# aymenboudhina/Multimodal_VQVAE_compression_audio_tactile

Measured on AMD Instinct MI355X. Metric: encode+VQ+decode token-frames/sec (1 frame = 13.33 ms of paired 24 kHz audio+tactile), higher is better.
Workload: dtype f32

## Files before the change

### multimodal_vqvae_compression_audio_tactile_amd/csrc/conv1d_mfma.hpp

```cpp
#pragma once
#include <hip/hip_runtime.h>
#include <stdio.h>
#include <stdlib.h>
#include <type_traits>
#include "det_math.hpp"
#include "kernels_small.hpp"

namespace mvq {

struct ConvArgs;
inline bool conv_dma_rows_ok(const ConvArgs& a);

__device__ __attribute__((aligned(16))) static const float g_zero16[4] = {0.0f, 0.0f, 0.0f, 0.0f};

int prof_begin(const char* kernel_name, double flops, hipStream_t s);
void prof_end(int idx, hipStream_t s);
bool prof_enabled();

typedef float f32x16 __attribute__((ext_vector_type(16)));
typedef float f32x4 __attribute__((ext_vector_type(4)));

struct ConvArgs {
    const float* x;
    const float* wp;
// ... 215 lines not shown
    static_assert(WAVES_M * WAVES_N == 4 || WAVES_M * WAVES_N == 8, "block is 4 or 8 waves");
    static_assert(KC % 2 == 0, "chunk K must be even (32x32x2 MFMA)");
    static_assert(BM % 4 == 0, "float4 weight staging");
};

template <int KS, int STRIDE, int DIL, int CK, int MT, int NT, int WAVES_M, int WAVES_N, int UPS, bool VEC>
struct ConvTile {
    using C = ConvCfg<KS, STRIDE, DIL, CK, MT, NT, WAVES_M, WAVES_N, UPS>;
    const float* wp; const float* xb; const float* Al;
    float* Ws; float* Xs;
    int tid, Tin, Cin, Mpad, m0, t_in0, g_al;
    bool snake_in;

    __device__ __forceinline__ void load_chunk(int chunk, f32x4 (&wreg)[C::W_PER_THREAD], f32x4 (&xv)[C::XV_PER_THREAD], float (&xs)[C::XS_PER_THREAD]) const
    {
        const int ci0 = chunk * CK;
        const float* wsrc = wp + (size_t)ci0 * KS * Mpad + m0;
#pragma unroll
        for (int u = 0; u < C::W_PER_THREAD; ++u) {
            int v = tid + u * C::NTHR;
            if (C::W_VEC % C::NTHR != 0) v = v < C::W_VEC ? v : C::W_VEC - 1;
            const int row = v / (C::BM / 4);
            const int c4 = v - row * (C::BM / 4);
            wreg[u] = *reinterpret_cast<const f32x4*>(wsrc + (size_t)row * Mpad + c4 * 4);
        }
        if (VEC) {
#pragma unroll
            for (int u = 0; u < C::XV_PER_THREAD; ++u) {
                int e = tid + u * C::NTHR;
                if (C::XV_TOTAL % C::NTHR != 0) e = e < C::XV_TOTAL ? e : C::XV_TOTAL - 1;
                const int cl = e / C::XV;
                const int v = e - cl * C::XV;
                const int g = g_al + 4 * v;
                const bool ok = g >= 0 && g < Tin;
                const int gc = ok ? g : 0;
                xv[u] = *reinterpret_cast<const f32x4*>(xb + (size_t)(ci0 + cl) * Tin + gc);
            }
        } else {
#pragma unroll
            for (int u = 0; u < C::XS_PER_THREAD; ++u) {
                int e = tid + u * C::NTHR;
                if (C::XS_TOTAL % C::NTHR != 0) e = e < C::XS_TOTAL ? e : C::XS_TOTAL - 1;
                const int cl = e / C::XT;
                const int xi = e - cl * C::XT;
                const int g = t_in0 + xi;
                const bool ok = g >= 0 && g < Tin;
                const int gc = ok ? g : 0;
                xs[u] = xb[(size_t)(ci0 + cl) * Tin + gc];
            }
        }
    }

    __device__ __forceinline__ void store_chunk(int chunk, int buf, const f32x4 (&wreg)[C::W_PER_THREAD],
                                                const f32x4 (&xv)[C::XV_PER_THREAD],
                                                const float (&xs)[C::XS_PER_THREAD]) const
    {
        const int ci0 = chunk * CK;
        float* wdst = Ws + buf * C::W_FLOATS;
        float* xdst = Xs + buf * C::X_FLOATS;
#pragma unroll
        for (int u = 0; u < C::W_PER_THREAD; ++u) {
            const int v = tid + u * C::NTHR;
            if (C::W_VEC % C::NTHR == 0 || v < C::W_VEC) *reinterpret_cast<f32x4*>(wdst + v * 4) = wreg[u];
        }
        if (VEC) {
#pragma unroll
            for (int u = 0; u < C::XV_PER_THREAD; ++u) {
                const int e = tid + u * C::NTHR;
                const int ec = (C::XV_TOTAL % C::NTHR != 0 && e >= C::XV_TOTAL) ? C::XV_TOTAL - 1 : e;
                const int cl = ec / C::XV;
                const int v = ec - cl * C::XV;
                const int g = g_al + 4 * v;
                const bool ok = g >= 0 && g < Tin;
                f32x4 q = xv[u];
                if (!ok) q = f32x4{0.0f, 0.0f, 0.0f, 0.0f};
                if (snake_in) {
                    const float al = Al[ci0 + cl], inv = Al[Cin + ci0 + cl];
                    q.x = det_snake(q.x, al, inv); q.y = det_snake(q.y, al, inv);
                    q.z = det_snake(q.z, al, inv); q.w = det_snake(q.w, al, inv);
                }
                if (C::XV_TOTAL % C::NTHR == 0 || e < C::XV_TOTAL)
                    *reinterpret_cast<f32x4*>(xdst + cl * C::XTP + 4 * v) = q;
            }
        } else {
#pragma unroll
            for (int u = 0; u < C::XS_PER_THREAD; ++u) {
                const int e = tid + u * C::NTHR;
                const int ec = (C::XS_TOTAL % C::NTHR != 0 && e >= C::XS_TOTAL) ? C::XS_TOTAL - 1 : e;
                const int cl = ec / C::XT;
                const int xi = ec - cl * C::XT;
                const int g = t_in0 + xi;
                float q = (g >= 0 && g < Tin) ? xs[u] : 0.0f;
                if (snake_in) q = det_snake(q, Al[ci0 + cl], Al[Cin + ci0 + cl]);
                if (C::XS_TOTAL % C::NTHR == 0 || e < C::XS_TOTAL) xdst[cl * C::XTP + xi] = q;
            }
        }
    }
};

template <int KS, int STRIDE, int DIL, int CK, int MT, int NT, int WAVES_M, int WAVES_N, int UPS, bool VEC, bool FUSE>
__device__ __forceinline__ void conv1d_mfma_body(const ConvArgs& a)
{
    using C = ConvCfg<KS, STRIDE, DIL, CK, MT, NT, WAVES_M, WAVES_N, UPS>;
    extern __shared__ __attribute__((aligned(16))) float smem[];
    float* const Ws = smem;
    float* const Xs = smem + 2 * C::W_FLOATS;
    float* const Ep = smem + (FUSE ? (a.dma ? C::LDS_FLOATS_FUSE_DMA : C::LDS_FLOATS_FUSE) : (a.dma ? C::LDS_FLOATS_DMA : C::LDS_FLOATS));
    constexpr int EP_MID = 2;
    float* const Al = Ep + 3 * C::BM;

    const int tid = threadIdx.x;
    const int lane = tid & 63;
    const int wave = tid >> 6;
    const int wm = wave / WAVES_N;
    const int wn = wave % WAVES_N;
    const int l31 = lane & 31;
    const int h = lane >> 5;

    int bx = blockIdx.x, by = blockIdx.y;
    if (a.row_fast) {
        const int xcd = bx & 7, j = bx >> 3;
        by = j % a.row_fast;
        bx = (j / a.row_fast) * 8 + xcd;
        if (bx >= a.n_tiles * a.B) return;
    }
    const int b = bx / a.n_tiles;
    const int tile_n = bx - b * a.n_tiles;
    const int n0 = a.n_base + tile_n * C::BN;
    const int m0 = by * C::BM;
    const int t_in0 = n0 * STRIDE - a.pad;
    const int g_al = t_in0 & ~3;
    const int shift = VEC ? (t_in0 - g_al) : 0;
    const int Cin = a.Cin;
    const int n_chunks = Cin / CK;
    const bool snake_in = a.alpha_in != nullptr;

    if (snake_in) {
        for (int c = tid; c < Cin; c += C::NTHR) {
            const float al = a.alpha_in[c];
            Al[c] = al;
            Al[Cin + c] = 1.0f / (al + 1e-9f);
        }
    }
    for (int r = tid; r < C::BM; r += C::NTHR) {
        int m = m0 + r;
        m = m < a.Mrows ? m : a.Mrows - 1;
        const int ch = m / (UPS ? UPS : 1);
        const float* tabs[4] = {a.alpha_out, a.y2 ? a.alpha2 : nullptr, FUSE ? a.alpha_mid : (a.dsn_src ? a.dsn_alpha : nullptr), nullptr};
#pragma unroll
        for (int k = 0; k < 3; ++k) {
            Ep[k * C::BM + r] = tabs[k] ? 1.0f / (tabs[k][ch] + 1e-9f) : 1.0f;
        }
    }

    ConvTile<KS, STRIDE, DIL, CK, MT, NT, WAVES_M, WAVES_N, UPS, VEC> tile;
    tile.wp = a.wp; tile.xb = a.x + (size_t)b * Cin * a.Tin; tile.Al = Al; tile.Ws = Ws; tile.Xs = Xs;
    tile.tid = tid; tile.Tin = a.Tin; tile.Cin = Cin; tile.Mpad = a.Mpad; tile.m0 = m0; tile.t_in0 = t_in0;
    tile.g_al = g_al; tile.snake_in = snake_in;

    f32x16 acc[MT][NT];
#pragma unroll
    for (int i = 0; i < MT; ++i)
#pragma unroll
        for (int j = 0; j < NT; ++j)
#pragma unroll
            for (int r = 0; r < 16; ++r) acc[i][j][r] = 0.0f;

    f32x4 wreg[C::W_PER_THREAD];
    f32x4 xv[C::XV_PER_THREAD];
    float xs[C::XS_PER_THREAD];

    constexpr int D_SAME = DIL;
    constexpr int D_CROSS = C::XTP - (KS - 1) * DIL;
    const int a_base = h * C::BM + wm * (MT * 32) + l31;
    const int b_base = (wn * (NT * 32) + l31) * STRIDE + shift;
    const int b_same = b_base + h * D_SAME;
    const int b_cross = b_base + h * D_CROSS;

    constexpr int NS = C::KC / 2;
    auto mfma_chunk = [&](int buf) __attribute__((always_inline)) {
        const float* wsrc = Ws + buf * C::W_FLOATS + a_base;
        const float* xs_same = Xs + buf * C::X_FLOATS + b_same;
        const float* xs_cross = Xs + buf * C::X_FLOATS + b_cross;
        float av[2][MT], bv[2][NT];
        auto load_step = [&](int st, int pb) __attribute__((always_inline)) {
            const int k0 = 2 * st;
            const int off0 = (k0 / KS) * C::XTP + (k0 % KS) * DIL;
            const bool cross = ((k0 + 1) / KS) != (k0 / KS);
            const float* xsp = cross ? xs_cross : xs_same;
#pragma unroll
            for (int i = 0; i < MT; ++i) av[pb][i] = wsrc[k0 * C::BM + i * 32];
#pragma unroll
            for (int j = 0; j < NT; ++j) bv[pb][j] = xsp[off0 + j * 32 * STRIDE];
        };
        load_step(0, 0);
#pragma unroll
        for (int s = 0; s < NS; ++s) {
            const int pb = s & 1;
            if (s + 1 < NS) load_step(s + 1, (s + 1) & 1);
#pragma unroll
            for (int i = 0; i < MT; ++i)
#pragma unroll
                for (int j = 0; j < NT; ++j)
                    acc[i][j] = __builtin_amdgcn_mfma_f32_32x32x2f32(av[pb][i], bv[pb][j], acc[i][j], 0, 0, 0);
            __builtin_amdgcn_sched_group_barrier(0x100, MT + NT, 0);
            __builtin_amdgcn_sched_group_barrier(0x008, MT * NT, 0);
        }
    };

    constexpr bool DMA_FITS = FUSE ? ((size_t)C::LDS_FLOATS_FUSE_DMA + 3 * C::BM) * 4 * 2 <= 160 * 1024 : (size_t)C::LDS_FLOATS_DMA * 4 <= 64 * 1024;
    bool use_dma = false;
    if constexpr (VEC && DMA_FITS) use_dma = a.dma != 0;
    if (use_dma) {
      if constexpr (VEC && DMA_FITS) {
        constexpr int NU = C::DMA_NU;
        constexpr int XP = C::XV4;
        constexpr int D_CROSS_D = XP - (KS - 1) * DIL;
        const int bd_same = b_base + h * D_SAME;
        const int bd_cross = b_base + h * D_CROSS_D;
        const float* src[NU];
        bool live[NU];
        long long step_b[NU];
#pragma unroll
        for (int u = 0; u < NU; ++u) {
            const int p = tid + u * C::NTHR;
            live[u] = p < C::DMA_NV;
            if (p < C::W_VEC) {
                const int row = p / (C::BM / 4), c4 = p - row * (C::BM / 4);
                src[u] = a.wp + (size_t)row * a.Mpad + m0 + c4 * 4;
                step_b[u] = (long long)CK * KS * a.Mpad;
            } else {
                const int q = (p < C::DMA_NV ? p : C::DMA_NV - 1) - C::W_VEC;
                const int cl = q / C::XV, v = q - cl * C::XV;
                const int g = g_al + 4 * v;
                bool ok = g >= 0 && g < a.Tin;
                const float* sp = tile.xb + (size_t)cl * a.Tin + g;
                long long st = (long long)CK * a.Tin;
                if (a.vp_seg) {
                    const int gg = ok ? g : 0;
                    const int seg = (int)__umulhi((unsigned)gg, a.vp_magic_in), pos = gg - seg * a.vp_per_in;
                    const int item = b * a.vp_seg + seg;
                    ok = ok && pos < a.vp_valid_in && item < a.vp_btrue;
                    sp = a.x + ((size_t)(ok ? item : 0) * a.Cin + cl) * a.vp_tin_phys + (ok ? pos : 0);
                    st = (long long)CK * a.vp_tin_phys;
                }
                src[u] = ok ? sp : g_zero16;
                step_b[u] = ok ? st : 0;
            }
        }
        const unsigned lds0 = (unsigned)(size_t)smem;
        const int wave_u = __builtin_amdgcn_readfirstlane(wave);
        const int n_issue = (NU - 1) * C::NTHR + wave_u * 64 < C::DMA_NV ? NU : NU - 1;
        constexpr int NFULL = C::DMA_NV / C::NTHR < NU ? C::DMA_NV / C::NTHR : NU;
        auto dma_chunk = [&](int stage) __attribute__((always_inline)) {
            const unsigned dst0 = lds0 + (unsigned)(stage * C::DMA_STAGE_FLOATS * 4) + (unsigned)(wave_u * 64 * 16);
            if constexpr (NFULL > 0) lds_dma_burst<NFULL, C::NTHR * 16>(src, dst0);
#pragma unroll
            for (int u = NFULL; u < NU; ++u) {
                if (live[u]) lds_dma_burst<1, C::NTHR * 16>(src + u, dst0 + (unsigned)(u * C::NTHR * 16));
            }
#pragma unroll
            for (int u = 0; u < NU; ++u) src[u] += step_b[u];
        };
        using AL = AsmOperandLoop<KS, STRIDE, DIL, C::BM, XP, MT, NT, NS>;
        auto mfma_chunk_asm = [&](int stage, bool issue_next, int next_stage) __attribute__((always_inline)) {
            const unsigned sb = lds0 + (unsigned)(stage * C::DMA_STAGE_FLOATS * 4);
            const unsigned a_addr = sb + (unsigned)(a_base * 4);
            const unsigned b_s = sb + (unsigned)((C::W_FLOATS + bd_same) * 4), b_c = sb + (unsigned)((C::W_FLOATS + bd_cross) * 4);
            float av0[MT], bv0[NT], av1[MT], bv1[NT];
            AL::template load_step<0>(av0, bv0, a_addr, b_s, b_c);
            if (issue_next) dma_chunk(next_stage);
            AL::template run_from<0>(acc, av0, bv0, av1, bv1, a_addr, b_s, b_c);
        };
        dma_chunk(0);
        if (n_chunks > 1) dma_chunk(1);
        int st_c = 0, st_n2 = 2;
        for (int c = 0; c < n_chunks; ++c) {
            if (c + 1 >= n_chunks) asm volatile("s_waitcnt vmcnt(0)" ::: "memory");
            else if (n_issue == NU) asm volatile("s_waitcnt vmcnt(%0)" :: "n"(NU) : "memory");
            else asm volatile("s_waitcnt vmcnt(%0)" :: "n"(NU - 1) : "memory");
            __syncthreads();
            mfma_chunk_asm(st_c, c + 2 < n_chunks, st_n2);
            st_c = st_c == 2 ? 0 : st_c + 1;
            st_n2 = st_n2 == 2 ? 0 : st_n2 + 1;
        }
      }
    } else {
    tile.load_chunk(0, wreg, xv, xs);
    __syncthreads();
    tile.store_chunk(0, 0, wreg, xv, xs);
    __syncthreads();
    for (int c = 0; c + 1 < n_chunks; ++c) {
        tile.load_chunk(c + 1, wreg, xv, xs);
        __builtin_amdgcn_sched_barrier(0);
        mfma_chunk(c & 1);
        __builtin_amdgcn_sched_barrier(0);
        tile.store_chunk(c + 1, (c + 1) & 1, wreg, xv, xs);
        __syncthreads();
    }
    mfma_chunk((n_chunks - 1) & 1);
    }

    const float* ep_bias = a.bias;
    if (FUSE) {
        float* const Ht = smem;
        __syncthreads();
#pragma unroll
        for (int i = 0; i < MT; ++i)
#pragma unroll
            for (int r = 0; r < 16; ++r) {
                const int row = (wm * MT + i) * 32 + (r & 3) + 8 * (r >> 2) + 4 * h;
                const float bv = a.bias ? a.bias[row] : 0.0f;
                const float al = a.alpha_mid[row], inv = Ep[EP_MID * C::BM + row];
#pragma unroll
                for (int j = 0; j < NT; ++j) {
                    Ht[row * C::BNP + (wn * NT + j) * 32 + l31] = det_snake(acc[i][j][r] + bv, al, inv);
                    acc[i][j][r] = 0.0f;
                }
            }
        __syncthreads();
        constexpr int K2 = C::BM / 2;
        constexpr int G = 8;
        static_assert(K2 % G == 0, "BM must be a multiple of 16");
        const float* w2 = a.w2p + (size_t)h * a.Mpad + wm * (MT * 32) + l31;
        const float* hsrc = Ht + h * C::BNP + wn * (NT * 32) + l31;
        float aw[2][G][MT];
#pragma unroll
        for (int g = 0; g < G; ++g)
#pragma unroll
            for (int i = 0; i < MT; ++i) aw[0][g][i] = w2[(size_t)(2 * g) * a.Mpad + i * 32];
#pragma unroll
        for (int grp = 0; grp < K2 / G; ++grp) {
            if (grp + 1 < K2 / G) {
#pragma unroll
                for (int g = 0; g < G; ++g)
#pragma unroll
                    for (int i = 0; i < MT; ++i)
                        aw[(grp + 1) & 1][g][i] = w2[(size_t)(2 * ((grp + 1) * G + g)) * a.Mpad + i * 32];
            }
#pragma unroll
            for (int g = 0; g < G; ++g) {
                const int s2 = grp * G + g;
                float bvv[NT];
#pragma unroll
                for (int j = 0; j < NT; ++j) bvv[j] = hsrc[2 * s2 * C::BNP + j * 32];
#pragma unroll
                for (int i = 0; i < MT; ++i)
#pragma unroll
                    for (int j = 0; j < NT; ++j)
                        acc[i][j] = __builtin_amdgcn_mfma_f32_32x32x2f32(aw[grp & 1][g][i], bvv[j], acc[i][j], 0, 0, 0);
            }
        }
        ep_bias = a.bias2;
    }

    const bool has_res = (UPS == 0) && a.residual != nullptr;
    const bool snake_out = a.alpha_out != nullptr;
    const bool do_tanh = a.act == 1;
    const bool do_gelu = a.act == 2;
    const bool direct = (UPS != 0) && (C::BM % (UPS ? UPS : 1) != 0);
    if (direct) {
#pragma unroll
        for (int i = 0; i < MT; ++i) {
#pragma unroll
            for (int r = 0; r < 16; ++r) {
                const int row = (r & 3) + 8 * (r >> 2) + 4 * h;
                const int m = m0 + (wm * MT + i) * 32 + row;
                const bool mok = m < a.Mrows;
                const int mc = mok ? m : a.Mrows - 1;
                const int co = mc / (UPS ? UPS : 1), rr = mc - co * (UPS ? UPS : 1);
                const float bv = ep_bias ? ep_bias[co] : 0.0f;
                const int lr = (wm * MT + i) * 32 + row;
                const float al = snake_out ? a.alpha_out[co] : 1.0f, inv = Ep[lr];
                const size_t rowoff = ((size_t)b * a.Cout + co) * a.Tout;
#pragma unroll
                for (int j = 0; j < NT; ++j) {
                    const int n = n0 + (wn * NT + j) * 32 + l31;
                    int t = n * (UPS ? UPS : 1) + rr - a.up_p;
                    bool ok = mok && n < a.Ncols && t >= 0 && (a.up_per_out ? true : t < a.Tout);
                    t = ok ? t : 0;
                    size_t ro = rowoff;
                    if (a.up_per_out) {
                        const int sg = (int)__umulhi((unsigned)t, a.up_magic);
                        t -= sg * a.up_per_out;
                        const int bb = b * a.up_seg + sg;
                        ok = ok && t < a.up_valid_out && bb < a.up_btrue;
                        ro = ((size_t)(ok ? bb : 0) * a.Cout + co) * a.Tout;
                        t = ok ? t : 0;
                    }
                    float v = acc[i][j][r] + bv;
                    const bool tail = a.tvalid && t >= a.tvalid;
                    if (ok && a.y2) a.y2[ro + t] = tail ? 0.0f : det_snake(v, a.alpha2[co], Ep[C::BM + lr]);
                    if (snake_out) v = det_snake(v, al, inv);
                    if (ok) a.y[ro + t] = tail ? 0.0f : v;
                }
            }
        }
        return;
    }

    float* const Ct = smem;
    constexpr int EHP = FUSE ? 1 : C::EH;
    constexpr int MTH = MT / EHP;
    constexpr int BMH = C::BM / EHP;
    auto tile_row_of = [&](int lrow, int pass) __attribute__((always_inline)) {
        if (EHP == 1) return lrow;
        const int g = lrow >> 5;
        return ((g / MTH) * MT + pass * MTH + (g % MTH)) * 32 + (lrow & 31);
    };
    auto epilogue_pass = [&](auto HP) __attribute__((always_inline)) {
    constexpr int hp = decltype(HP)::value;
    __syncthreads();
#pragma unroll
    for (int il = 0; il < MTH; ++il)
#pragma unroll
        for (int r = 0; r < 16; ++r) {
            const int row = (wm * MTH + il) * 32 + (r & 3) + 8 * (r >> 2) + 4 * h;
#pragma unroll
            for (int j = 0; j < NT; ++j) Ct[row * C::BNP + (wn * NT + j) * 32 + l31] = acc[hp * MTH + il][j][r];
        }
    constexpr int NVQ = BMH * C::BN / 4;
    constexpr bool PRE_RES = (UPS == 0) && (NVQ % C::NTHR == 0) && (NVQ / C::NTHR <= 16);
    constexpr int RES_IT = PRE_RES ? NVQ / C::NTHR : 1;
    constexpr int CQ = C::CQ, JN = C::JN;
    constexpr bool REG = PRE_RES && C::REG_GEOM && (BMH % C::RSTEP == 0);
    constexpr int RSTEP = REG ? C::RSTEP : 1;
    const bool reg_ok = REG && !(a.y2 && a.alpha_out);
    const int q_c0 = REG ? tid % CQ : 0, q_r0 = REG ? tid / CQ : 0;
    auto reg_k = [&](int it, int pass) __attribute__((always_inline)) {
        const int lr = (it / JN) * RSTEP;
        if (EHP == 1) return lr;
        const int g = lr >> 5;
        return ((g / MTH) * MT + pass * MTH + (g % MTH)) * 32 + (lr & 31);
    };
    const size_t blk_off = a.vp_seg ? ((size_t)b * a.vp_seg * a.Cout + m0) * a.Tout : ((size_t)b * a.Cout + m0) * a.Tout + n0;
    const unsigned q_t0 = (unsigned)(q_r0 * a.Tout);
    bool q_nok[JN];
    unsigned q_col[JN];
    int q_vpos[JN];
#pragma unroll
    for (int j = 0; j < JN; ++j) {
        const int n = n0 + 4 * (q_c0 + j * CQ);
        q_nok[j] = n < a.Ncols;
        q_col[j] = 4u * (q_c0 + j * CQ);
        q_vpos[j] = 0;
        if (a.vp_seg) {
            const int nn = q_nok[j] ? n : 0;
            const int seg = (int)__umulhi((unsigned)nn, a.vp_magic_out), pos = nn - seg * a.vp_per_out;
            q_nok[j] = q_nok[j] && b * a.vp_seg + seg < a.vp_btrue && pos < a.Tout;
            q_col[j] = (unsigned)(seg * a.Cout * a.Tout + pos);
            q_vpos[j] = pos;
        }
    }
    f32x4 res_q[RES_IT];
    if (PRE_RES && has_res && a.ovec4) {
        bool pre_done = false;
        if constexpr (REG) if (reg_ok) {
            pre_done = true;
            const float* resb = a.residual + blk_off;
#pragma unroll
            for (int it = 0; it < RES_IT; ++it) {
                const int k = reg_k(it, hp), j = it % JN;
                const bool ok = q_nok[j] && m0 + q_r0 + k < a.Mrows;
                res_q[it] = *reinterpret_cast<const f32x4*>(resb + (ok ? q_t0 + (unsigned)(k * a.Tout) + q_col[j] : 0u));
            }
        }
        if (!pre_done) {
#pragma unroll
            for (int it = 0; it < RES_IT; ++it) {
                const int e = tid + it * C::NTHR;
                const int row = e / (C::BN / 4);
                const int c4 = e - row * (C::BN / 4);
                const int m = m0 + tile_row_of(row, hp), n = n0 + 4 * c4;
                const bool ok = m < a.Mrows && n < a.Ncols;
                const size_t off = ((size_t)b * a.Cout + (ok ? m : 0)) * a.Tout + (ok ? n : 0);
                res_q[it] = *reinterpret_cast<const f32x4*>(a.residual + off);
            }
        }
    }
    float* const Tb = smem + (FUSE ? C::CT_FLOATS : C::CTH_FLOATS);
    if (reg_ok && hp == 0) {
        const float* const ax = a.y2 ? a.alpha2 : a.alpha_out;
        for (int r = tid; r < C::BM; r += C::NTHR) {
            int m = m0 + r;
            m = m < a.Mrows ? m : a.Mrows - 1;
            Tb[r] = ep_bias ? ep_bias[m] : 0.0f;
            Tb[C::BM + r] = ax ? ax[m] : 1.0f;
        }
    }
    __syncthreads();
    auto tile_row = [&](int lrow) __attribute__((always_inline)) { return tile_row_of(lrow, hp); };

    if (UPS == 0) {
        if (a.ovec4) {
            constexpr int NV = BMH * C::BN / 4;
            auto quad = [&](int e, int it) __attribute__((always_inline)) {
                const int row = e / (C::BN / 4);
                const int c4 = e - row * (C::BN / 4);
                const int m = m0 + tile_row(row), n = n0 + 4 * c4;
                if (m < a.Mrows && n < a.Ncols) {
                    const float bv = ep_bias ? ep_bias[m] : 0.0f;
                    f32x4 v = *reinterpret_cast<const f32x4*>(Ct + row * C::BNP + 4 * c4);
                    const size_t off = ((size_t)b * a.Cout + m) * a.Tout + n;
                    v.x = v.x + bv; v.y = v.y + bv; v.z = v.z + bv; v.w = v.w + bv;
                    if (a.dsn_src) {
                        const float ad = a.dsn_alpha[m], id = Ep[2 * C::BM + tile_row(row)];
                        const f32x4 sv = *reinterpret_cast<const f32x4*>(a.dsn_src + off);
                        v.x = v.x * det_dsnake(sv.x, ad, id); v.y = v.y * det_dsnake(sv.y, ad, id);
                        v.z = v.z * det_dsnake(sv.z, ad, id); v.w = v.w * det_dsnake(sv.w, ad, id);
                    }
                    if (has_res) {
                        const f32x4 rv = PRE_RES ? res_q[PRE_RES ? it : 0] : *reinterpret_cast<const f32x4*>(a.residual + off);
                        v.x = v.x + rv.x; v.y = v.y + rv.y; v.z = v.z + rv.z; v.w = v.w + rv.w;
                    }
                    int nz = (a.tvalid && n + 4 > a.tvalid) ? n + 4 - a.tvalid : 0;
                    if (a.tper) {
                        const int nn = n - (int)__umulhi((unsigned)n, a.tper_magic) * a.tper;
                        nz = nn + 4 > a.tper_valid ? (nn >= a.tper_valid ? 4 : nn + 4 - a.tper_valid) : 0;
                    }
                    if (a.y2) {
                        const float a2 = a.alpha2[m], i2 = Ep[C::BM + tile_row(row)];
                        f32x4 w = {det_snake(v.x, a2, i2), det_snake(v.y, a2, i2), det_snake(v.z, a2, i2), det_snake(v.w, a2, i2)};
                        if (nz > 0) { w.w = 0.0f; if (nz > 1) w.z = 0.0f; if (nz > 2) w.y = 0.0f; if (nz > 3) w.x = 0.0f; }
                        *reinterpret_cast<f32x4*>(a.y2 + off) = w;
                    }
                    if (snake_out) {
                        const float al = a.alpha_out[m], inv = Ep[tile_row(row)];
                        v.x = det_snake(v.x, al, inv); v.y = det_snake(v.y, al, inv);
                        v.z = det_snake(v.z, al, inv); v.w = det_snake(v.w, al, inv);
                    }
                    if (do_tanh) { v.x = det_tanh(v.x); v.y = det_tanh(v.y); v.z = det_tanh(v.z); v.w = det_tanh(v.w); }
                    if (do_gelu) { v.x = det_gelu(v.x); v.y = det_gelu(v.y); v.z = det_gelu(v.z); v.w = det_gelu(v.w); }
                    if (nz > 0) { v.w = 0.0f; if (nz > 1) v.z = 0.0f; if (nz > 2) v.y = 0.0f; if (nz > 3) v.x = 0.0f; }
                    *reinterpret_cast<f32x4*>(a.y + off) = v;
                }
            };
            bool quads_done = false;
            if constexpr (REG) if (reg_ok) {
                quads_done = true;
                int nz[JN];
#pragma unroll
                for (int j = 0; j < JN; ++j) {
                    const int n = n0 + 4 * (q_c0 + j * CQ);
                    nz[j] = (a.tvalid && n + 4 > a.tvalid) ? n + 4 - a.tvalid : 0;
                    if (a.tper) {
                        const int nn = n - (int)__umulhi((unsigned)n, a.tper_magic) * a.tper;
                        nz[j] = nn + 4 > a.tper_valid ? (nn >= a.tper_valid ? 4 : nn + 4 - a.tper_valid) : 0;
                    }
                    if (a.vp_seg) {
                        const int pp = q_vpos[j];
                        nz[j] = pp + 4 > a.vp_valid_out ? (pp >= a.vp_valid_out ? 4 : pp + 4 - a.vp_valid_out) : 0;
                    }
                }
                float* const yb = a.y + blk_off;
                float* const y2b = a.y2 ? a.y2 + blk_off : nullptr;
                const float* const dsb = a.dsn_src ? a.dsn_src + blk_off : nullptr;
                const float* const ctq = Ct + q_r0 * C::BNP + 4 * q_c0;
                const float* const tbq = Tb + q_r0;
                const float* const epq = Ep + q_r0;
                auto reg_quads = [&](auto MODE_) __attribute__((always_inline)) {
                    constexpr int MODE = decltype(MODE_)::value;
                    const bool f_dsn = MODE == 0 ? (a.dsn_src != nullptr) : false;
                    const bool f_res = MODE == 0 ? has_res : (MODE == 1 || MODE == 2 || MODE == 5);
                    const bool f_y2 = MODE == 0 ? (a.y2 != nullptr) : (MODE == 1 || MODE == 4);
                    const bool f_so = MODE == 0 ? snake_out : (MODE == 2 || MODE == 3);
                    const bool f_tanh = MODE == 0 ? do_tanh : false;
                    const bool f_gelu = MODE == 0 ? do_gelu : false;
#pragma unroll
                    for (int it = 0; it < RES_IT; ++it) {
                        const int k = reg_k(it, hp), j = it % JN;
                        const int trow = q_r0 + k;
                        if (q_nok[j] && m0 + trow < a.Mrows) {
                            const unsigned toff = q_t0 + (unsigned)(k * a.Tout) + q_col[j];
                            const float bv = tbq[k];
                            f32x4 v = *reinterpret_cast<const f32x4*>(ctq + (it / JN) * RSTEP * C::BNP + 4 * CQ * j);
                            v.x = v.x + bv; v.y = v.y + bv; v.z = v.z + bv; v.w = v.w + bv;
                            if (f_dsn) {
                                const float ad = a.dsn_alpha[m0 + trow], id = epq[2 * C::BM + k];
                                const f32x4 sv = *reinterpret_cast<const f32x4*>(dsb + toff);
                                v.x = v.x * det_dsnake(sv.x, ad, id); v.y = v.y * det_dsnake(sv.y, ad, id);
                                v.z = v.z * det_dsnake(sv.z, ad, id); v.w = v.w * det_dsnake(sv.w, ad, id);
                            }
                            if (f_res) {
                                const f32x4 rv = res_q[it];
                                v.x = v.x + rv.x; v.y = v.y + rv.y; v.z = v.z + rv.z; v.w = v.w + rv.w;
                            }
                            const int z = nz[j];
                            if (f_y2) {
                                const float a2 = tbq[C::BM + k], i2 = epq[C::BM + k];
                                f32x4 w = {det_snake(v.x, a2, i2), det_snake(v.y, a2, i2), det_snake(v.z, a2, i2), det_snake(v.w, a2, i2)};
                                if (z > 0) { w.w = 0.0f; if (z > 1) w.z = 0.0f; if (z > 2) w.y = 0.0f; if (z > 3) w.x = 0.0f; }
                                *reinterpret_cast<f32x4*>(y2b + toff) = w;
                            }
                            if (f_so) {
                                const float al = tbq[C::BM + k], inv = epq[k];
                                v.x = det_snake(v.x, al, inv); v.y = det_snake(v.y, al, inv);
                                v.z = det_snake(v.z, al, inv); v.w = det_snake(v.w, al, inv);
                            }
                            if (f_tanh) { v.x = det_tanh(v.x); v.y = det_tanh(v.y); v.z = det_tanh(v.z); v.w = det_tanh(v.w); }
                            if (f_gelu) { v.x = det_gelu(v.x); v.y = det_gelu(v.y); v.z = det_gelu(v.z); v.w = det_gelu(v.w); }
                            if (z > 0) { v.w = 0.0f; if (z > 1) v.z = 0.0f; if (z > 2) v.y = 0.0f; if (z > 3) v.x = 0.0f; }
                            *reinterpret_cast<f32x4*>(yb + toff) = v;
                        }
                    }
                };
                const bool plain = !a.dsn_src && !do_tanh && !do_gelu;
                const bool hy2 = a.y2 != nullptr;
                if (!plain) reg_quads(std::integral_constant<int, 0>{});
                else if (has_res && hy2 && !snake_out) reg_quads(std::integral_constant<int, 1>{});
                else if (has_res && !hy2 && snake_out) reg_quads(std::integral_constant<int, 2>{});
                else if (!has_res && !hy2 && snake_out) reg_quads(std::integral_constant<int, 3>{});
                else if (!has_res && hy2 && !snake_out) reg_quads(std::integral_constant<int, 4>{});
                else if (has_res && !hy2 && !snake_out) reg_quads(std::integral_constant<int, 5>{});
                else if (!has_res && !hy2 && !snake_out) reg_quads(std::integral_constant<int, 6>{});
                else reg_quads(std::integral_constant<int, 0>{});
            }
            if (quads_done) {
            } else if (PRE_RES) {
#pragma unroll
                for (int it = 0; it < RES_IT; ++it) quad(tid + it * C::NTHR, it);
            } else {
#pragma unroll 4
                for (int e = tid; e < NV; e += C::NTHR) quad(e, 0);
            }
        } else {
            constexpr int NE = BMH * C::BN;
#pragma unroll 4
            for (int e = tid; e < NE; e += C::NTHR) {
                const int row = e / C::BN;
                const int col = e - row * C::BN;
                const int m = m0 + tile_row(row), n = n0 + col;
                if (m < a.Mrows && n < a.Ncols) {
                    const size_t off = ((size_t)b * a.Cout + m) * a.Tout + n;
                    float v = Ct[row * C::BNP + col] + (ep_bias ? ep_bias[m] : 0.0f);
                    const int lr = tile_row(row);
                    if (a.dsn_src) v = v * det_dsnake(a.dsn_src[off], a.dsn_alpha[m], Ep[2 * C::BM + lr]);
                    if (has_res) v = v + a.residual[off];
                    bool tail = a.tvalid && n >= a.tvalid;
                    if (a.tper) tail = n - (int)__umulhi((unsigned)n, a.tper_magic) * a.tper >= a.tper_valid;
                    if (a.y2) a.y2[off] = tail ? 0.0f : det_snake(v, a.alpha2[m], Ep[C::BM + lr]);
                    if (snake_out) v = det_snake(v, a.alpha_out[m], Ep[lr]);
                    if (do_tanh) v = det_tanh(v);
                    if (do_gelu) v = det_gelu(v);
                    a.y[off] = tail ? 0.0f : v;
                }
            }
        }
    } else {
        constexpr int S = UPS ? UPS : 1;
        const int run = C::BN * S;
        const int nco = BMH / S;
        const int t_base = n0 * S - a.up_p;
        const int total = nco * run;
        auto shuffle_one = [&](int col, int tl) __attribute__((always_inline)) {
            const int nl = tl / S, rr = tl - nl * S;
            const int co = (m0 + tile_row(col * S)) / S;
            int t = t_base + tl;
            bool ok = co < a.Cout && n0 + nl < a.Ncols && t >= 0 && (a.up_per_out ? true : t < a.Tout);
            int bb = b;
            if (ok && a.up_per_out) {
                const int sg = (int)__umulhi((unsigned)t, a.up_magic);
                t -= sg * a.up_per_out;
                bb = b * a.up_seg + sg;
                ok = t < a.up_valid_out && bb < a.up_btrue;
            }
            if (ok) {
                float v = Ct[(col * S + rr) * C::BNP + nl] + (ep_bias ? ep_bias[co] : 0.0f);
                const size_t off = ((size_t)bb * a.Cout + co) * a.Tout + t;
                const bool tail = a.tvalid && t >= a.tvalid;
                const int lr = tile_row(col * S);
                if (a.y2) a.y2[off] = tail ? 0.0f : det_snake(v, a.alpha2[co], Ep[C::BM + lr]);
                if (snake_out) v = det_snake(v, a.alpha_out[co], Ep[lr]);
                a.y[off] = tail ? 0.0f : v;
            }
        };
        const bool up_quads = a.ovec4 && (C::BN * S) % 4 == 0 && (a.up_per_out == 0 || (a.up_per_out % 4 == 0 && a.up_valid_out % 4 == 0));
        if (up_quads) {
            const int lead = (4 - (t_base & 3)) & 3;
            const int QF = (run - lead) / 4;
            const int totq = nco * QF;
            for (int e = tid; e < totq; e += C::NTHR) {
                const int col = e / QF;
                const int tl0 = lead + 4 * (e - col * QF);
                const int co = (m0 + tile_row(col * S)) / S;
                int t = t_base + tl0;
                const int nl_last = (tl0 + 3) / S;
                bool ok = co < a.Cout && n0 + nl_last < a.Ncols && t >= 0 && (a.up_per_out ? true : t + 3 < a.Tout);
                int bb = b;
                if (ok && a.up_per_out) {
                    const int sg = (int)__umulhi((unsigned)t, a.up_magic);
                    t -= sg * a.up_per_out;
                    bb = b * a.up_seg + sg;
                    ok = t < a.up_valid_out && bb < a.up_btrue;
                } else if (!ok && co < a.Cout) {
#pragma unroll
                    for (int i = 0; i < 4; ++i) shuffle_one(col, tl0 + i);
                    continue;
                }
                if (!ok) continue;
                const float bv = ep_bias ? ep_bias[co] : 0.0f;
                f32x4 v;
#pragma unroll
                for (int i = 0; i < 4; ++i) {
                    const int tl = tl0 + i, nl = tl / S, rr = tl - nl * S;
                    v[i] = Ct[(col * S + rr) * C::BNP + nl] + bv;
                }
                const size_t off = ((size_t)bb * a.Cout + co) * a.Tout + t;
                const int lr = tile_row(col * S);
                int nz = (a.tvalid && t + 4 > a.tvalid) ? t + 4 - a.tvalid : 0;
                nz = nz > 4 ? 4 : nz;
                if (a.y2) {
                    const float a2 = a.alpha2[co], i2 = Ep[C::BM + lr];
                    f32x4 w = {det_snake(v.x, a2, i2), det_snake(v.y, a2, i2), det_snake(v.z, a2, i2), det_snake(v.w, a2, i2)};
                    if (nz > 0) { w.w = 0.0f; if (nz > 1) w.z = 0.0f; if (nz > 2) w.y = 0.0f; if (nz > 3) w.x = 0.0f; }
                    *reinterpret_cast<f32x4*>(a.y2 + off) = w;
                }
                if (snake_out) {
                    const float al = a.alpha_out[co], inv = Ep[lr];
                    v.x = det_snake(v.x, al, inv); v.y = det_snake(v.y, al, inv); v.z = det_snake(v.z, al, inv); v.w = det_snake(v.w, al, inv);
                }
                if (nz > 0) { v.w = 0.0f; if (nz > 1) v.z = 0.0f; if (nz > 2) v.y = 0.0f; if (nz > 3) v.x = 0.0f; }
                *reinterpret_cast<f32x4*>(a.y + off) = v;
            }
            const int rest = run - 4 * QF;
            for (int e = tid; e < nco * rest; e += C::NTHR) {
                const int col = e / rest, r = e - col * rest;
                shuffle_one(col, r < lead ? r : 4 * QF + r);
            }
        } else
        for (int e = tid; e < total; e += C::NTHR) {
            const int col = e / run;
            const int tl = e - col * run;
            const int nl = tl / S, rr = tl - nl * S;
            const int co = (m0 + tile_row(col * S)) / S;
            int t = t_base + tl;
            bool ok = co < a.Cout && n0 + nl < a.Ncols && t >= 0 && (a.up_per_out ? true : t < a.Tout);
            int bb = b;
            if (ok && a.up_per_out) {
                const int sg = (int)__umulhi((unsigned)t, a.up_magic);
                t -= sg * a.up_per_out;
                bb = b * a.up_seg + sg;
                ok = t < a.up_valid_out && bb < a.up_btrue;
            }
            if (ok) {
                float v = Ct[(col * S + rr) * C::BNP + nl] + (ep_bias ? ep_bias[co] : 0.0f);
                const size_t off = ((size_t)bb * a.Cout + co) * a.Tout + t;
                const bool tail = a.tvalid && t >= a.tvalid;
                const int lr = tile_row(col * S);
                if (a.y2) a.y2[off] = tail ? 0.0f : det_snake(v, a.alpha2[co], Ep[C::BM + lr]);
                if (snake_out) v = det_snake(v, a.alpha_out[co], Ep[lr]);
                a.y[off] = tail ? 0.0f : v;
            }
        }
    }
    };
    epilogue_pass(std::integral_constant<int, 0>{});
    if constexpr (EHP == 2) epilogue_pass(std::integral_constant<int, 1>{});
    static_assert(EHP == 1 || EHP == 2, "one or two epilogue passes");
}

template <int KS, int STRIDE, int DIL, int CK, int MT, int NT, int WAVES_M, int WAVES_N, int UPS>
__global__ __attribute__((amdgpu_flat_work_group_size(1, 64 * WAVES_M * WAVES_N),
                          amdgpu_waves_per_eu(ConvCfg<KS, STRIDE, DIL, CK, MT, NT, WAVES_M, WAVES_N, UPS>::MIN_WPE)))
void conv1d_mfma_kernel(const ConvArgs a)
{
    if (a.vec4) conv1d_mfma_body<KS, STRIDE, DIL, CK, MT, NT, WAVES_M, WAVES_N, UPS, true, false>(a);
    else conv1d_mfma_body<KS, STRIDE, DIL, CK, MT, NT, WAVES_M, WAVES_N, UPS, false, false>(a);
}

template <int DIL, int CK, int MT, int NT, int WAVES_M, int WAVES_N>
__global__ __attribute__((amdgpu_flat_work_group_size(1, 64 * WAVES_M * WAVES_N),
                          amdgpu_waves_per_eu(ConvCfg<7, 1, DIL, CK, MT, NT, WAVES_M, WAVES_N, 0>::MIN_WPE_FUSE)))
void residual_unit_kernel(const ConvArgs a)
{
    if (a.vec4) conv1d_mfma_body<7, 1, DIL, CK, MT, NT, WAVES_M, WAVES_N, 0, true, true>(a);
    else conv1d_mfma_body<7, 1, DIL, CK, MT, NT, WAVES_M, WAVES_N, 0, false, true>(a);
}

template <int DIL, int CK, int MT, int NT, int WAVES_M, int WAVES_N>
inline hipError_t launch_residual_unit(const ConvArgs& a_in, hipStream_t stream)
{
    using C = ConvCfg<7, 1, DIL, CK, MT, NT, WAVES_M, WAVES_N, 0>;
    ConvArgs a = a_in;
    if (a.Cin % CK != 0 || a.Cout != C::BM || a.Cin != C::BM || a.Mpad != C::BM) return hipErrorInvalidValue;
    if (a.name_out) {
        snprintf(a.name_out, a.name_len, "residual_unit_kernel<%d, %d, %d, %d, %d, %d>", DIL, CK, MT, NT, WAVES_M, WAVES_N);
        return hipSuccess;
    }
    a.n_tiles = (a.Ncols + C::BN - 1) / C::BN;
    a.vec4 = (a.Tin % 4 == 0) && ((reinterpret_cast<uintptr_t>(a.x) & 15) == 0);
    a.ovec4 = (a.Tout % 4 == 0) && ((reinterpret_cast<uintptr_t>(a.y) & 15) == 0) &&
              ((reinterpret_cast<uintptr_t>(a.residual) & 15) == 0);
    a.dma = (conv_dma_rows_ok(a) && ((size_t)C::LDS_FLOATS_FUSE_DMA + 3 * C::BM) * 4 * 2 <= 160 * 1024) ? 1 : 0;
    const size_t lds = a.dma ? (size_t)C::LDS_FLOATS_FUSE_DMA * 4 + (size_t)3 * C::BM * 4
                             : (size_t)C::LDS_FLOATS_FUSE * 4 + (size_t)3 * C::BM * 4 + (size_t)2 * a.Cin * 4;
    auto kern = residual_unit_kernel<DIL, CK, MT, NT, WAVES_M, WAVES_N>;
    {
        static BigLdsOptIn opt;
        const hipError_t e = opt.ensure(reinterpret_cast<const void*>(kern));
        if (e != hipSuccess) return e;
    }
    dim3 grid((unsigned)(a.n_tiles * a.B), 1);
    int pi = -1;
    if (prof_enabled()) {
        char nm[96];
        snprintf(nm, sizeof(nm), "residual_unit_kernel<%d, %d, %d, %d, %d, %d>", DIL, CK, MT, NT, WAVES_M, WAVES_N);
        const int cols = a.tvalid > 0 ? a.tvalid : a.Ncols;
        pi = prof_begin(nm, 2.0 * a.Cin * a.Cout * 8.0 * cols * a.B, stream);
    }
    hipLaunchKernelGGL(kern, grid, dim3(C::NTHR), lds, stream, a);
    prof_end(pi, stream);
    return hipGetLastError();
}

template <int KS, int STRIDE, int DIL, int CK, int MT, int NT, int WAVES_M, int WAVES_N, int UPS>
inline hipError_t launch_conv1d_mfma(const ConvArgs& a_in, hipStream_t stream)
{
    using C = ConvCfg<KS, STRIDE, DIL, CK, MT, NT, WAVES_M, WAVES_N, UPS>;
    ConvArgs a = a_in;
    if (a.Cin % CK != 0 || a.Mpad % C::BM != 0) return hipErrorInvalidValue;
    if (C::XALIGNED && (a.pad != 0 || a.n_base % 4 != 0)) return hipErrorInvalidValue;
    if (a.name_out) {
        snprintf(a.name_out, a.name_len, "conv1d_mfma_kernel<%d, %d, %d, %d, %d, %d, %d, %d, %d>", KS, STRIDE, DIL, CK, MT, NT,
                 WAVES_M, WAVES_N, UPS);
        return hipSuccess;
    }
    a.n_tiles = (a.Ncols - a.n_base + C::BN - 1) / C::BN;
    if (a.n_tiles_max > 0 && a.n_tiles > a.n_tiles_max) a.n_tiles = a.n_tiles_max;
    a.vec4 = (a.Tin % 4 == 0) && ((reinterpret_cast<uintptr_t>(a.x) & 15) == 0);
    a.ovec4 = (a.Tout % 4 == 0) && ((reinterpret_cast<uintptr_t>(a.y) & 15) == 0) &&
              (!a.residual || (reinterpret_cast<uintptr_t>(a.residual) & 15) == 0) &&
              (!a.y2 || (reinterpret_cast<uintptr_t>(a.y2) & 15) == 0) &&
              (!a.dsn_src || (reinterpret_cast<uintptr_t>(a.dsn_src) & 15) == 0);
    a.dma = (conv_dma_rows_ok(a) && (size_t)C::LDS_FLOATS_DMA * 4 <= 64 * 1024) ? 1 : 0;
    const size_t lds = (a.dma ? (size_t)C::LDS_FLOATS_DMA * 4 : (size_t)C::LDS_FLOATS * 4 + (a.alpha_in ? (size_t)2 * a.Cin * 4 : 0)) + (size_t)3 * C::BM * 4;
    auto kern = conv1d_mfma_kernel<KS, STRIDE, DIL, CK, MT, NT, WAVES_M, WAVES_N, UPS>;
    {
        static BigLdsOptIn opt;
        const hipError_t e = opt.ensure(reinterpret_cast<const void*>(kern));
        if (e != hipSuccess) return e;
    }
    if (lds > 160 * 1024) return hipErrorInvalidValue;
    if (a.vp_seg) {
        constexpr int EHP_ = C::EH, NVQ_ = (C::BM / EHP_) * C::BN / 4;
        constexpr bool REG_ = C::REG_GEOM && (NVQ_ % C::NTHR == 0) && (NVQ_ / C::NTHR <= 16) && ((C::BM / EHP_) % C::RSTEP == 0);
        if (!REG_ || UPS != 0 || !a.dma || !a.ovec4 || (a.y2 && a.alpha_out)) return hipErrorInvalidValue;
    }
    const unsigned gx = (unsigned)(a.n_tiles * a.B), R = (unsigned)((a.Mrows + C::BM - 1) / C::BM);
    dim3 grid(gx, R);
    a.row_fast = 0;
    if (R > 1 && (size_t)a.Cin * KS * a.Mpad * sizeof(float) <= ((size_t)5 << 19)) {
        a.row_fast = (int)R;
        grid = dim3(((gx + 7) / 8) * 8 * R, 1);
    }
    int pi = -1;
    if (prof_enabled()) {
        char nm[96];
        snprintf(nm, sizeof(nm), "conv1d_mfma_kernel<%d, %d, %d, %d, %d, %d, %d, %d, %d>", KS, STRIDE, DIL, CK, MT, NT, WAVES_M, WAVES_N, UPS);
        int last = a.n_base + a.n_tiles * C::BN;
        int lim = a.Ncols;
        if (UPS > 0 && !a.up_per_out) lim = a.Ncols - 1;
        else if (a.tvalid > 0) lim = a.tvalid;
        if (last > lim) last = lim;
        double cols = last > a.n_base ? last - a.n_base : 0;
        if (a.tper) cols *= (double)a.tper_valid / a.tper;
        if (a.vp_seg) cols *= ((double)a.vp_valid_out / a.vp_per_out) * ((double)a.vp_btrue / ((double)a.B * a.vp_seg));
        if (a.up_per_out) cols *= (double)a.up_valid_out / a.up_per_out;
        pi = prof_begin(nm, 2.0 * a.Cin * KS * a.Mrows * cols * a.B, stream);
    }
    hipLaunchKernelGGL(kern, grid, dim3(C::NTHR), lds, stream, a);
    prof_end(pi, stream);
    return hipGetLastError();
}

inline bool conv_dma_rows_ok(const ConvArgs& a)
{
    static const bool off = getenv("MVQ_NO_DMA") != nullptr;
    return !off && !a.alpha_in && a.Tin % 4 == 0 && (reinterpret_cast<uintptr_t>(a.x) & 15) == 0;
}

inline int conv_tile_bm(int mrows)
{
    if (mrows % 128 == 0) return 128;
    if (mrows % 96 == 0) return 96;
    if (mrows % 64 == 0) return 64;
    return mrows > 96 ? 128 : (mrows > 64 ? 96 : 64);
}
inline int conv_mpad(int mrows) { const int bm = conv_tile_bm(mrows); return (mrows + bm - 1) / bm * bm; }

inline int conv_tail_width(const ConvArgs& a)
{
    if (a.n_base != 0 || a.n_tiles_max != 0) return 0;
    if ((long)a.B * ((a.Mrows + 127) / 128) < 128) return 0;
    const int full = a.Ncols / 128, rem = a.Ncols % 128;
    if (full == 0 || rem == 0 || rem > 96) return 0;
    const int w = rem <= 64 ? 64 : 96;
    return (128 - w) * 100 >= (full + 1) * 128 ? w : 0;
}

inline bool conv_underfilled(const ConvArgs& a)
{
    return (long)a.B * ((a.Ncols + 127) / 128) * ((a.Mrows + 127) / 128) < 160;
}
inline bool conv_prefer_small_tiles(const ConvArgs& a)
{
    if (a.Mpad % 64 != 0) return false;
    if (a.vp_seg) return false;
    const long big = (long)a.B * ((a.Ncols + 127) / 128) * ((a.Mrows + 127) / 128);
    if (big < 160) return true;
    if (big >= 600) return false;
    const long small = 4 * big;
    const double fill_big = (double)big / (double)((big + 255) / 256 * 256);
    const double fill_small = (double)small / (double)((small + 255) / 256 * 256);
    return 0.85 * fill_small > fill_big;
}

}
```

Baseline: 60380.

## Prefetch fused residual-unit operands earlier to hide global load latency

```diff
diff --git a/multimodal_vqvae_compression_audio_tactile_amd/csrc/conv1d_mfma.hpp b/multimodal_vqvae_compression_audio_tactile_amd/csrc/conv1d_mfma.hpp
--- a/multimodal_vqvae_compression_audio_tactile_amd/csrc/conv1d_mfma.hpp
+++ b/multimodal_vqvae_compression_audio_tactile_amd/csrc/conv1d_mfma.hpp
@@ -391,6 +391,14 @@
             Ep[k * C::BM + r] = tabs[k] ? 1.0f / (tabs[k][ch] + 1e-9f) : 1.0f;
         }
     }
+    constexpr bool MID_TB = FUSE && (size_t)3 * C::DMA_STAGE_FLOATS <= (size_t)C::CT_FLOATS &&
+                            (size_t)C::STAGE_FLOATS <= (size_t)C::CT_FLOATS && C::TB_FLOATS == 2 * C::BM;
+    if constexpr (MID_TB) {
+        for (int r = tid; r < C::BM; r += C::NTHR) {
+            smem[C::CT_FLOATS + r] = a.bias ? a.bias[r] : 0.0f;
+            smem[C::CT_FLOATS + C::BM + r] = a.alpha_mid[r];
+        }
+    }
 
     ConvTile<KS, STRIDE, DIL, CK, MT, NT, WAVES_M, WAVES_N, UPS, VEC> tile;
     tile.wp = a.wp; tile.xb = a.x + (size_t)b * Cin * a.Tin; tile.Al = Al; tile.Ws = Ws; tile.Xs = Xs;
@@ -444,6 +452,18 @@
                     acc[i][j] = __builtin_amdgcn_mfma_f32_32x32x2f32(av[pb][i], bv[pb][j], acc[i][j], 0, 0, 0);
             __builtin_amdgcn_sched_group_barrier(0x100, MT + NT, 0);
             __builtin_amdgcn_sched_group_barrier(0x008, MT * NT, 0);
+        }
+    };
+
+    constexpr int G1 = 8;
+    float aw[2][G1][MT];
+    const float* const w2 = FUSE ? a.w2p + (size_t)h * a.Mpad + wm * (MT * 32) + l31 : nullptr;
+    auto w2_first_group = [&]() __attribute__((always_inline)) {
+        if constexpr (FUSE) {
+#pragma unroll
+            for (int g = 0; g < G1; ++g)
+#pragma unroll
+                for (int i = 0; i < MT; ++i) aw[0][g][i] = w2[(size_t)(2 * g) * a.Mpad + i * 32];
         }
     };
 
@@ -519,6 +539,7 @@
             else if (n_issue == NU) asm volatile("s_waitcnt vmcnt(%0)" :: "n"(NU) : "memory");
             else asm volatile("s_waitcnt vmcnt(%0)" :: "n"(NU - 1) : "memory");
             __syncthreads();
+            if constexpr (FUSE) if (c + 1 == n_chunks) w2_first_group();
             mfma_chunk_asm(st_c, c + 2 < n_chunks, st_n2);
             st_c = st_c == 2 ? 0 : st_c + 1;
             st_n2 = st_n2 == 2 ? 0 : st_n2 + 1;
@@ -537,20 +558,65 @@
         tile.store_chunk(c + 1, (c + 1) & 1, wreg, xv, xs);
         __syncthreads();
     }
+    if constexpr (FUSE) {
+        w2_first_group();
+        __builtin_amdgcn_sched_barrier(0);
+    }
     mfma_chunk((n_chunks - 1) & 1);
     }
 
     const float* ep_bias = a.bias;
+    constexpr int F_NVQ = C::BM * C::BN / 4;
+    constexpr bool F_PRE = FUSE && UPS == 0 && (F_NVQ % C::NTHR == 0) && (F_NVQ / C::NTHR <= 16) && C::REG_GEOM &&
+                           (C::BM % C::RSTEP == 0);
+    constexpr int F_IT = F_PRE ? F_NVQ / C::NTHR : 1;
+    f32x4 res_pre[F_IT];
+    float tb_pre[2] = {0.0f, 1.0f};
+    const bool f_tb = F_PRE && !(a.y2 && a.alpha_out);
+    const bool f_res = f_tb && a.residual != nullptr && a.ovec4;
+    auto epi_prefetch = [&]() __attribute__((always_inline)) {
+        if constexpr (F_PRE) {
+            static_assert(C::BM <= C::NTHR, "one row-table entry per thread");
+            if (f_res) {
+                constexpr int CQ = C::CQ, JN = C::JN, RSTEP = C::RSTEP;
+                const int q_c0 = tid % CQ, q_r0 = tid / CQ;
+                const float* resb = a.residual + (((size_t)b * a.Cout + m0) * a.Tout + n0);
+#pragma unroll
+                for (int it = 0; it < F_IT; ++it) {
+                    const int k = (it / JN) * RSTEP, j = it % JN;
+                    const unsigned col = 4u * (q_c0 + j * CQ);
+                    const bool ok = n0 + (int)col < a.Ncols && m0 + q_r0 + k < a.Mrows;
+                    res_pre[it] = *reinterpret_cast<const f32x4*>(resb + (ok ? (unsigned)(q_r0 * a.Tout) + (unsigned)(k * a.Tout) + col : 0u));
+                }
+            }
+            if (f_tb) {
+                const int r = tid < C::BM ? tid : C::BM - 1;
+                const float* ax = a.y2 ? a.alpha2 : a.alpha_out;
+                const float vb = (a.bias2 ? a.bias2 : a.alpha_mid)[m0 + r];
+                const float va = (ax ? ax : a.alpha_mid)[m0 + r];
+                tb_pre[0] = a.bias2 ? vb : 0.0f;
+                tb_pre[1] = ax ? va : 1.0f;
+            }
+        }
+    };
     if (FUSE) {
         float* const Ht = smem;
+        const float* const Tbm = smem + C::CT_FLOATS;
         __syncthreads();
 #pragma unroll
         for (int i = 0; i < MT; ++i)
 #pragma unroll
             for (int r = 0; r < 16; ++r) {
                 const int row = (wm * MT + i) * 32 + (r & 3) + 8 * (r >> 2) + 4 * h;
-                const float bv = a.bias ? a.bias[row] : 0.0f;
-                const float al = a.alpha_mid[row], inv = Ep[EP_MID * C::BM + row];
+                float bv, al;
+                if constexpr (MID_TB) {
+                    bv = Tbm[row];
+                    al = Tbm[C::BM + row];
+                } else {
+                    bv = a.bias ? a.bias[row] : 0.0f;
+                    al = a.alpha_mid[row];
+                }
+                const float inv = Ep[EP_MID * C::BM + row];
 #pragma unroll
                 for (int j = 0; j < NT; ++j) {
                     Ht[row * C::BNP + (wn * NT + j) * 32 + l31] = det_snake(acc[i][j][r] + bv, al, inv);
@@ -559,15 +625,9 @@
             }
         __syncthreads();
         constexpr int K2 = C::BM / 2;
-        constexpr int G = 8;
-        static_assert(K2 % G == 0, "BM must be a multiple of 16");
-        const float* w2 = a.w2p + (size_t)h * a.Mpad + wm * (MT * 32) + l31;
+        constexpr int G = G1;
+        static_assert(K2 % G == 0 && K2 / G >= 2, "BM must be a multiple of 16, at least 32");
         const float* hsrc = Ht + h * C::BNP + wn * (NT * 32) + l31;
-        float aw[2][G][MT];
-#pragma unroll
-        for (int g = 0; g < G; ++g)
-#pragma unroll
-            for (int i = 0; i < MT; ++i) aw[0][g][i] = w2[(size_t)(2 * g) * a.Mpad + i * 32];
 #pragma unroll
         for (int grp = 0; grp < K2 / G; ++grp) {
             if (grp + 1 < K2 / G) {
@@ -577,6 +637,7 @@
                     for (int i = 0; i < MT; ++i)
                         aw[(grp + 1) & 1][g][i] = w2[(size_t)(2 * ((grp + 1) * G + g)) * a.Mpad + i * 32];
             }
+            if (grp + (MT > 1 ? 1 : 2) == K2 / G) epi_prefetch();
 #pragma unroll
             for (int g = 0; g < G; ++g) {
                 const int s2 = grp * G + g;
@@ -696,12 +757,18 @@
         bool pre_done = false;
         if constexpr (REG) if (reg_ok) {
             pre_done = true;
+            if constexpr (FUSE) {
+                static_assert(RES_IT == F_IT, "fused unit: the 1x1-phase prefetch covers this pass");
+#pragma unroll
+                for (int it = 0; it < RES_IT; ++it) res_q[it] = res_pre[it];
+            } else {
             const float* resb = a.residual + blk_off;
 #pragma unroll
             for (int it = 0; it < RES_IT; ++it) {
                 const int k = reg_k(it, hp), j = it % JN;
                 const bool ok = q_nok[j] && m0 + q_r0 + k < a.Mrows;
                 res_q[it] = *reinterpret_cast<const f32x4*>(resb + (ok ? q_t0 + (unsigned)(k * a.Tout) + q_col[j] : 0u));
+            }
             }
         }
         if (!pre_done) {
@@ -718,7 +785,9 @@
         }
     }
     float* const Tb = smem + (FUSE ? C::CT_FLOATS : C::CTH_FLOATS);
-    if (reg_ok && hp == 0) {
+    if (FUSE && reg_ok && hp == 0) {
+        if (tid < C::BM) { Tb[tid] = tb_pre[0]; Tb[C::BM + tid] = tb_pre[1]; }
+    } else if (reg_ok && hp == 0) {
         const float* const ax = a.y2 ? a.alpha2 : a.alpha_out;
         for (int r = tid; r < C::BM; r += C::NTHR) {
             int m = m0 + r;
@@ -1022,6 +1091,7 @@
     using C = ConvCfg<7, 1, DIL, CK, MT, NT, WAVES_M, WAVES_N, 0>;
     ConvArgs a = a_in;
     if (a.Cin % CK != 0 || a.Cout != C::BM || a.Cin != C::BM || a.Mpad != C::BM) return hipErrorInvalidValue;
+    if (a.vp_seg || a.tper || a.dsn_src) return hipErrorInvalidValue;
     if (a.name_out) {
         snprintf(a.name_out, a.name_len, "residual_unit_kernel<%d, %d, %d, %d, %d, %d>", DIL, CK, MT, NT, WAVES_M, WAVES_N);
         return hipSuccess;
```

Result: no change. 60620, median of 6 (+0.4%).
